# symek/facedeform

Hardware: AMD Instinct MI355X
Metric: deformed Mverts/sec at 256 ctrl pts, 1/2/4/8 MI355X vs host-CPU ref (higher is better)
Workload: dtype f32

## Files before the change

### facedeform_amd/csrc/fd_capi.hip

```cpp
#include <atomic>
#include <cstdarg>
#include <cstdio>
#include <cstdlib>
#include <cstring>
#include <new>

#include "fd_internal.h"

using namespace fd;

struct GraphKey {
    int M, kind, term, nparams;
    double params[4];
    const void *A, *rest, *rec32;
};

struct fd_batch;
struct fd_ctx {
    int device = 0;
    hipStream_t own_stream = nullptr;
    hipStream_t stream_ = nullptr;
    int eval_precision = FD_EVAL_FP32;
    int eval_variant = 0;
    int output = FD_OUTPUT_POSITION;
// ... 1631 lines not shown
    hipError_t e = launch_deform_batch(args, b->n, stream);
    if (e != hipSuccess) { batch_err(b, "launch_deform_batch failed: %s", hipGetErrorString(e)); return FD_E_DEVICE; }
    return FD_OK;
}

static int shared_applies(fd_batch *b, const char *who, float *const *d_P_out, int *ek_out)
{
    fd_ctx *c0 = b->ctxs[0];
    const int ek = eval_kind(c0);
    *ek_out = ek;
    bool fast = (ek == FD_KERNEL_THIN_PLATE || ek == FD_KERNEL_GAUSSIAN || ek == FD_KERNEL_GAUSSIAN_QNN) && round_up(c0->M, kRecPad) >= 32;
    for (int i = 0; i < b->n; ++i) {
        fd_ctx *c = b->ctxs[i];
        if (!d_P_out[i]) { batch_err(b, "%s: NULL output array for context %d", who, i); return FD_E_INVALID; }
        if (!c->built && !c->build_pending) { batch_err(b, "%s: context %d has no built model", who, i); return FD_E_NOT_BUILT; }
        if (!c->rest_src || c->rest_src != c0->rest_src || !same_model(c, c0)) {
            batch_err(b, "%s: the contexts must share one rest rig (fd_batch_set_points_dev with the "
                         "same rest array for all), kernel and term; context %d does not", who, i);
            return FD_E_INVALID;
        }
        if (c->output != c0->output) { batch_err(b, "%s: context %d has another fd_set_output setting than context 0", who, i); return FD_E_INVALID; }
        if (c->eval_precision != FD_EVAL_FP32 || c->eval_variant > 0 || record_layers(c) != 0) fast = false;
    }
    return fast ? 1 : 0;
}

static bool make_event(hipEvent_t *ev)
{
    if (*ev) return true;
    if (hipEventCreateWithFlags(ev, hipEventDisableTiming) != hipSuccess) { (void)hipGetLastError(); *ev = nullptr; return false; }
    return true;
}

static int shared_pack(fd_batch *b, hipStream_t stream, int ek, float *const *d_P_out, float *const *d_falloff_out)
{
    fd_ctx *c0 = b->ctxs[0];
    const int si = b->packed_valid ? (b->cur_set ^ 1) : 0;
    fd_batch::SharedSet &st = b->sets[si];
    SharedDeformArgs a{};
    a.N = 1; a.Mpad = round_up(c0->M, kRecPad); a.nF = b->n; a.kind = ek; a.ctiles = c0->d_tiles16;
    a.falloff_out = d_falloff_out;
    int rc;
    if (!b->lean && (rc = batch_poll(b))) return rc;
    for (int i = 0; i < b->n; ++i) {
        fd_ctx *c = b->ctxs[i];
        a.rec32[i] = c->d_rec32; a.model[i] = c->d_model; a.P_out[i] = d_P_out[i]; a.centres[i] = c->d_centres;
        if ((rc = order_after_batch(c, stream))) { batch_err(b, "context %d: %s", i, c->err); return rc; }
    }
    {
        bool one_build = c0->rig_build_id != 0;
        for (int i = 1; i < b->n && one_build; ++i) one_build = b->ctxs[i]->rig_build_id == c0->rig_build_id;
        if (one_build) for (int i = 1; i < b->n; ++i) a.centres[i] = a.centres[0];
    }
    const size_t wb = shared_wtile_bytes(a.Mpad, a.nF), fb = shared_frame_bytes(a.nF);
    if (wb > st.cap_wtiles || fb > st.cap_frames) {
        if (st.d_wtiles) (void)hipFree(st.d_wtiles);
        if (st.d_frames) (void)hipFree(st.d_frames);
        st.d_wtiles = st.d_frames = nullptr; st.cap_wtiles = st.cap_frames = 0; st.eval_pending = false;
        if (hipMalloc(&st.d_wtiles, wb) != hipSuccess || hipMalloc(&st.d_frames, fb) != hipSuccess) {
            (void)hipGetLastError();
            batch_err(b, "shared-rig evaluation: scratch allocation (%zu bytes) failed", wb + fb);
            return FD_E_NOMEM;
        }
        st.cap_wtiles = wb; st.cap_frames = fb;
    }
    if (st.eval_pending && st.eval_done && hipStreamWaitEvent(stream, st.eval_done, 0) != hipSuccess) {
        batch_err(b, "shared-rig evaluation: hipStreamWaitEvent failed: %s", hipGetErrorString(hipGetLastError()));
        return FD_E_DEVICE;
    }
    st.eval_pending = false;
    a.wtiles = st.d_wtiles; a.frames = st.d_frames;
    a.packed_ev = b->lean ? nullptr : (make_event(&st.packed_ev) ? st.packed_ev : nullptr);
    b->consumed_override = nullptr;
    a.mode = 1;
    a.M = c0->M;
    if (b->h_mismatch && hipHostGetDevicePointer((void **)&a.mismatch, b->h_mismatch, 0) != hipSuccess) { (void)hipGetLastError(); a.mismatch = nullptr; }
    hipError_t e = launch_deform_shared(a, stream);
    if (e != hipSuccess) { batch_err(b, "launch_deform_shared (pack) failed: %s", hipGetErrorString(e)); return FD_E_DEVICE; }
    b->cur_set = si;
    b->packed_valid = b->lean || st.packed_ev != nullptr;
    b->prepared = true;
    for (int i = 0; i < b->n; ++i) {
        b->prep_P_out[i] = d_P_out[i]; b->prep_fall[i] = d_falloff_out ? d_falloff_out[i] : nullptr;
        b->prep_gen[i] = b->ctxs[i]->model_gen;
    }
    b->prep_has_fall = d_falloff_out != nullptr;
    return FD_OK;
}

int fd_batch_prepare_shared(fd_batch *b, void *hip_stream, float *const *d_P_out, float *const *d_falloff_out)
{
    if (!b || !d_P_out) return FD_E_INVALID;
    fd_ctx *c0 = b->ctxs[0];
    int rc = use_device(c0);
    if (rc) { batch_err(b, "%s", c0->err); return rc; }
    hipStream_t stream = hip_stream ? (hipStream_t)hip_stream : cur_stream(c0);
    int ek = 0;
    const int applies = shared_applies(b, "fd_batch_prepare_shared", d_P_out, &ek);
    if (applies < 0) return applies;
    if (applies == 0) return FD_OK;
    return shared_pack(b, stream, ek, d_P_out, d_falloff_out);
}

int fd_batch_deform_shared_dev(fd_batch *b, void *hip_stream, int64_t N, const float *d_P_in, float *const *d_P_out,
                               const float *d_dist2, float *const *d_falloff_out, const float *d_tu,
                               const float *d_tv, const float *d_nrm, float radius2, float falloffrate)
{
    if (!b || !d_P_out) return FD_E_INVALID;
    if (N < 0 || (N > 0 && !d_P_in)) { batch_err(b, "fd_batch_deform_shared_dev: bad N / P_in"); return FD_E_INVALID; }
// ... 12 lines not shown
        rc = fd_batch_deform_dev(b, hip_stream, N, pin, d_P_out, d_dist2 ? pd2 : nullptr, d_falloff_out, d_tu ? ptu : nullptr,
                                 d_tu ? ptv : nullptr, d_tu ? pnr : nullptr, radius2, falloffrate);
        if (rc == FD_OK && make_event(&b->fallback_ev)) {
            if (hipEventRecord(b->fallback_ev, stream) != hipSuccess) { (void)hipGetLastError(); rc = FD_E_DEVICE; }
            b->packed_valid = false;
            b->consumed_override = nullptr;
        }
        return rc;
    }
    bool reuse = b->prepared && b->prep_has_fall == (d_falloff_out != nullptr);
    for (int i = 0; reuse && i < b->n; ++i)
        reuse = b->prep_P_out[i] == d_P_out[i] && (!d_falloff_out || b->prep_fall[i] == d_falloff_out[i]) &&
                b->prep_gen[i] == b->ctxs[i]->model_gen;
    if (reuse) {
        if (!b->lean && (rc = batch_poll(b))) return rc;
        if (!b->prepared) reuse = false;
        for (int i = 0; reuse && i < b->n; ++i)
            if ((rc = order_after_batch(b->ctxs[i], stream))) { batch_err(b, "context %d: %s", i, b->ctxs[i]->err); return rc; }
    }
    if (reuse) {
        fd_batch::SharedSet &ps = b->sets[b->cur_set];
        if (!b->lean && ps.packed_ev && hipStreamWaitEvent(stream, ps.packed_ev, 0) != hipSuccess) {
            batch_err(b, "fd_batch_deform_shared_dev: hipStreamWaitEvent failed: %s", hipGetErrorString(hipGetLastError()));
            return FD_E_DEVICE;
        }
    } else if ((rc = shared_pack(b, stream, ek, d_P_out, d_falloff_out))) {
        return rc;
    }
    fd_batch::SharedSet &st = b->sets[b->cur_set];
    SharedDeformArgs a{};
    a.N = N; a.P_in = d_P_in; a.dist2 = d_dist2; a.tu = d_tu; a.tv = d_tv; a.nrm = d_nrm;
    a.radius2 = radius2; a.falloffrate = falloffrate;
    a.Mpad = round_up(c0->M, kRecPad); a.nF = b->n;
    a.ctiles = c0->d_tiles16;
    a.kind = ek;
    a.falloff_out = d_falloff_out;
    for (int i = 0; i < b->n; ++i) { a.rec32[i] = b->ctxs[i]->d_rec32; a.model[i] = b->ctxs[i]->d_model; a.P_out[i] = d_P_out[i]; }
    a.wtiles = st.d_wtiles; a.frames = st.d_frames;
    a.packed_ev = nullptr;
    a.mode = 2;
    a.delta_out = c0->output == FD_OUTPUT_DISPLACEMENT;
    a.max_wgs = b->eval_cus;
    hipError_t e = launch_deform_shared(a, stream);
    if (e != hipSuccess) { batch_err(b, "launch_deform_shared failed: %s", hipGetErrorString(e)); return FD_E_DEVICE; }
    if (b->lean) {
        st.eval_done = b->ev1;
        st.eval_pending = true;
    } else if (make_event(&st.eval_ev)) {
        st.eval_done = st.eval_ev;
        if (hipEventRecord(st.eval_ev, stream) != hipSuccess) { (void)hipGetLastError(); st.eval_pending = false; }
        else st.eval_pending = true;
    } else {
        (void)hipStreamSynchronize(stream);
    }
    return FD_OK;
}

int fd_batch_deform_vectors_shared_dev(fd_batch *b, void *hip_stream, int64_t N, const float *d_P_in, float *const *d_P_out,
                                       const float *d_dist2, float *const *d_falloff_out, const float *d_tu, const float *d_tv,
                                       const float *d_nrm, float radius2, float falloffrate, const fd_batch_vectors *vec)
{
    if (!b || !d_P_out) return FD_E_INVALID;
    const char *who = "fd_batch_deform_vectors_shared_dev";
    if (vec && vec->struct_size < (int)sizeof(fd_batch_vectors)) {
        batch_err(b, "%s: vec->struct_size is %d, must be sizeof(fd_batch_vectors) = %d", who, vec->struct_size, (int)sizeof(fd_batch_vectors));
        return FD_E_INVALID;
    }
    const bool want = vec && (vec->N || vec->N_out || vec->tu || vec->tu_out || vec->tv || vec->tv_out || vec->jacobian);
    if (!want)
        return fd_batch_deform_shared_dev(b, hip_stream, N, d_P_in, d_P_out, d_dist2, d_falloff_out, d_tu, d_tv, d_nrm, radius2, falloffrate);
// ... 176 lines not shown
```

### facedeform_amd/csrc/fd_eval_shared.hip

```cpp
#include <cstdio>
#include <cstdlib>

#include <type_traits>

#include "fd_eval_common.h"

namespace fd {

namespace {

typedef _Float16 f16x8 __attribute__((ext_vector_type(8)));
typedef _Float16 f16x2 __attribute__((ext_vector_type(2)));

constexpr int kSharedThreads = 512;
constexpr int kWideWaves = 8;
constexpr size_t kSharedLdsBudget = 158 * 1024;

constexpr int kGaussShift = 10;
constexpr bool shared_dense(int nF) { return nF > 12; }
constexpr int shared_tiles(int nF) { return shared_dense(nF) ? 3 * ((nF + 15) / 16) : (nF + 3) / 4; }
constexpr int shared_slots(int nT, bool dense) { return dense ? nT / 3 * 16 : nT * 4; }

struct SharedFrame {
    float inv_scale;
    int built;
    int pad[2];
    float *P_out, *falloff_out;
};
static_assert(sizeof(SharedFrame) == 32, "frame record");

struct SharedOut {
    float *P_out[kMaxBatch];
// ... 536 lines not shown
                }
                if (fout) __builtin_nontemporal_store(fall, (float FD_GLOBAL *)((char FD_GLOBAL *)(fout + 4ull * (uint64_t)vbase) + off4));
                store_pos3_nt(dstP, base[0] + disp[0] * fall, base[1] + disp[1] * fall, base[2] + disp[2] * fall);
            }
        }
        FD_SSTAMP(3)
    };
    int grp = blockIdx.x;
    bool built_here = true;
#pragma unroll
    for (int q = 0; q < kTabRegs; ++q) {
        const int idx = 64 * q + lane;
        if (idx < kSlots * 8 && (idx & 7) == 1) built_here = built_here && tab[q] != 0u;
    }
    if (p.fast && __all(built_here)) {
        const int nfull = (int)(p.N / kSharedThreads);
        for (; grp < nfull; grp += gridDim.x) do_group(grp, std::true_type{});
    }
    for (; grp < ngroups; grp += gridDim.x) do_group(grp, std::false_type{});
    if (stamp && lane == 0) {
        for (int q = 0; q < 4; ++q) p.stamps[wave * 8 + q] = st_acc[q];
    }
#undef FD_SSTAMP
}


typedef float f32x16 __attribute__((ext_vector_type(16)));
constexpr bool shared_wide(int nF, int kind) { (void)kind; return nF > 16; }
constexpr int kWideSlots = 32;
constexpr int wide_slots(int nF) { return (nF + 3) / 4 * 4; }
constexpr int wide_tiles(int nslot) { return (3 * nslot + 31) / 32; }
constexpr int wide_w16(int nt) { return nt * 2 * 2 * 64; }

__global__ __launch_bounds__(256) void k_pack_shared_wide(const SharedSlots slots, const SharedOut out, int nF, int nslot, int Mpad,
                                                           uint4 *wtiles, SharedFrame *frames, const MfmaTileH *ctiles, int gauss, int layout)
{
    const int kb = blockIdx.x, T = blockIdx.y, nkb = gridDim.x, NT = gridDim.y;
    const int w16 = wide_w16(NT);
    const size_t poly_at = (size_t)nkb * w16, copy_at = poly_at + (size_t)NT * 64;
    if (T == 0) {
        uint2 *dst = reinterpret_cast<uint2 *>(wtiles + copy_at) + (size_t)kb * 128;
        if (gauss) {
            if (threadIdx.x < 32) {
                const int centre = 32 * kb + (int)threadIdx.x;
                wtiles[copy_at + (size_t)kb * 64 + threadIdx.x] =
                    centre < Mpad ? *reinterpret_cast<const uint4 *>(&slots.rec32[0][centre]) : make_uint4(0u, 0u, 0u, 0u);
            }
        } else if (layout == 1) {
            if (threadIdx.x < 64) {
                const int lane = threadIdx.x, h = lane >> 5, r = lane & 31;
                const int tile = 2 * kb + (r >> 4);
                uint4 v = make_uint4(0u, 0u, 0u, 0u);
                if (tile < Mpad / 16) {
                    const unsigned *a0 = ctiles[tile].a[16 * (2 * h) + (r & 15)], *a1 = ctiles[tile].a[16 * (2 * h + 1) + (r & 15)];
                    v = make_uint4(a0[0], a0[1], a1[0], a1[1]);
                }
                wtiles[copy_at + (size_t)kb * 64 + lane] = v;
            }
        } else if (threadIdx.x < 128) {
            const int i = threadIdx.x >> 6, lane = threadIdx.x & 63, h = lane >> 5, r = lane & 31;
            const int tile = 2 * kb + (r >> 4);
            uint2 v = make_uint2(0u, 0u);
            if (tile < Mpad / 16) { const unsigned *a = ctiles[tile].a[16 * (2 * i + h) + (r & 15)]; v = make_uint2(a[0], a[1]); }
            dst[threadIdx.x] = v;
        }
        if (kb == 0 && threadIdx.x == 255) {
            const float *nn = slots.model[0]->norm32;
            wtiles[copy_at + (size_t)nkb * 64] = make_uint4(__float_as_uint(nn[0]), __float_as_uint(nn[1]), __float_as_uint(nn[2]), __float_as_uint(nn[3]));
        }
    }
    __shared__ float s_scale[kWideSlots];
    {
        const int f = threadIdx.x >> 3, l = threadIdx.x & 7;
        float m = 0.f;
        if (f < nslot) {
            m = slots.model[f]->wmax32;
        }
        for (int off = 4; off >= 1; off >>= 1) m = fmaxf(m, __shfl_xor(m, off));
        const bool same_rig = (kb == 0 && T == 0) ? rig_matches(slots, f, nslot, l, 8) : true;
        if (l == 0) {
            int k = 0;
            if (m > 0.f && m < INFINITY) k = 13 - (__builtin_amdgcn_frexp_expf(m) - 1);
            k = k < -100 ? -100 : (k > 100 ? 100 : k);
            s_scale[f] = ldexpf(1.f, k);
            if (kb == 0 && T == 0) {
                SharedFrame fr;
                fr.inv_scale = ldexpf(1.f, -k - (gauss ? kGaussShift : 0));
                fr.built = (f < nslot && same_rig && slots.model[f]->terminationtype == 1) ? 1 : 0;
                fr.pad[0] = fr.pad[1] = 0;
                fr.P_out = f < nslot ? out.P_out[f] : nullptr;
                fr.falloff_out = f < nslot ? out.falloff_out[f] : nullptr;
                frames[f] = fr;
            }
        }
    }
    __syncthreads();
    if (threadIdx.x >= 128) return;
    const int s = threadIdx.x >> 6, lane = threadIdx.x & 63, h = lane >> 5;
    int f, c;
    if (layout == 1) {
        const int rho = lane & 31, k = 16 * T + 4 * (rho >> 3) + (rho & 3);
        f = 2 * (k / 3) + ((rho >> 2) & 1); c = k % 3;
    } else {
        const int row = 32 * T + (lane & 31);
        f = row / 3; c = row % 3;
    }
    const bool live = f < nslot;
    const float sc = live ? s_scale[f] : 0.f;
    f16x8 hi, lo;
#pragma unroll
    for (int m = 0; m < 8; ++m) {
        const int centre = 32 * kb + 8 * (2 * s + (m >> 2)) + 4 * h + (m & 3);
        float w = 0.f;
        if (live && centre < Mpad) {
            const Rec32 r = slots.rec32[f][centre];
            w = (c == 0 ? r.wx : (c == 1 ? r.wy : r.wz)) * sc;
        }
        const _Float16 hh = (_Float16)w;
        hi[m] = hh;
        lo[m] = (_Float16)(w - (float)hh);
    }
    uint4 *dst = wtiles + (size_t)kb * w16 + (size_t)((T * 2 + s) * 2) * 64;
    dst[lane] = __builtin_bit_cast(uint4, hi);
    dst[64 + lane] = __builtin_bit_cast(uint4, lo);
    if (kb == 0 && s == 0) {
        f16x8 pt;
#pragma unroll
        for (int m = 0; m < 8; ++m) {
            const int coef = h == 0 ? (m < 5 ? m : m - 4) : (m == 0 ? 4 : (m < 6 ? m - 1 : -1));
            const bool want_lo = h == 1 && m >= 1;
            float w = 0.f;
            if (live && coef >= 0) w = slots.model[f]->poly32[5 * c + coef] * sc;
            const _Float16 hh = (_Float16)w;
            pt[m] = want_lo ? (_Float16)(w - (float)hh) : hh;
        }
        wtiles[poly_at + (size_t)T * 64 + lane] = __builtin_bit_cast(uint4, pt);
    }
}

constexpr int kWideVpm = 3;
constexpr int kW1Vpm = 3;

template <bool GAUSS, int NT, int NSLOT>
__global__ __launch_bounds__(64 * kWideWaves) __attribute__((amdgpu_waves_per_eu(kWideWaves / 4, kWideWaves / 4)))
void k_deform32_tps_shared_wide(const SharedParams p, int ngroups)
{
    constexpr int WAVES = kWideWaves, THREADS = 64 * WAVES;
    static_assert(NSLOT % 4 == 0 && NSLOT <= kWideSlots && 3 * NSLOT <= 32 * NT, "frame slots in fours, three rows each");
    constexpr int kWideW16 = wide_w16(NT);
    constexpr int TV = 2;
    constexpr int kSlots = kWideSlots;
    extern __shared__ __attribute__((aligned(16))) char smem[];
    SharedFrame *s_frames = reinterpret_cast<SharedFrame *>(smem);
    uint4 *s_poly = reinterpret_cast<uint4 *>(smem + sizeof(SharedFrame) * (size_t)kSlots);
    uint2 *s_ct = reinterpret_cast<uint2 *>(s_poly + NT * 64);
    uint4 *s_w = reinterpret_cast<uint4 *>(s_ct + (size_t)128 * p.kchunk);
    uint64_t *s_ftab = reinterpret_cast<uint64_t *>(s_w + (size_t)kWideW16 * p.kchunk);
    unsigned *s_ticket = reinterpret_cast<unsigned *>(s_ftab + 512);
    const int tid = threadIdx.x;
    const int lane = tid & 63;
    const int wave = __builtin_amdgcn_readfirstlane(tid >> 6);
    const int h = lane >> 5, j = lane & 31;
    const float n0 = p.norm[0], n1 = p.norm[1], n2 = p.norm[2];
    const float inv_s = p.norm[3];
    const bool resident = p.nkb <= p.kchunk;
    const unsigned long long st_t0 = p.stamps ? __builtin_amdgcn_s_memtime() : 0, st_r0 = p.stamps ? __builtin_amdgcn_s_memrealtime() : 0;
    f32x16 zero16;
#pragma unroll
    for (int r = 0; r < 16; ++r) zero16[r] = 0.f;

// ... 347 lines not shown
    int ru = dynamic ? round_taken : 0;
    nxt = load_raw(unit_group(u) < ngroups ? unit_global(u) : 0, std::false_type{});
    settle(nxt);
    if (fast_ok) {
        while (unit_group(u) < nfull) {
            const int un = next_unit(u);
            const int run = dynamic ? round_taken : ru + 1;
            do_group(u, un, ru, std::true_type{});
            u = un; ru = run;
        }
    }
    while (unit_group(u) < ngroups) {
        const int un = next_unit(u);
        const int run = dynamic ? round_taken : ru + 1;
        do_group(u, un, ru, std::false_type{});
        u = un; ru = run;
    }
    if (stamp && lane == 0 && wave < 8) {
        for (int q = 0; q < 4; ++q) p.stamps[wave * 8 + q] = st_acc[q];
        p.stamps[wave * 8 + 4] = __builtin_amdgcn_s_memtime() - st_t0;
        p.stamps[wave * 8 + 5] = __builtin_amdgcn_s_memrealtime() - st_r0;
    }
    if (p.stamps != nullptr && lane == 0 && wave < 8 && blockIdx.x < kMaxCUs) {
        p.stamps[64 + ((size_t)blockIdx.x * 8 + wave) * 2] = st_r0;
        p.stamps[64 + ((size_t)blockIdx.x * 8 + wave) * 2 + 1] = __builtin_amdgcn_s_memrealtime();
    }
#undef FD_SSTAMP
}

constexpr int kW1Waves = 12;
constexpr int kW1Unit = 32;
constexpr size_t w1_fixed_lds(int nt) { return sizeof(SharedFrame) * (size_t)kWideSlots + 32 * 16 + (size_t)nt * 64 * 16 + 256 * sizeof(uint64_t) + 16; }

template <bool GAUSS, int NT, int NSLOT>
__global__ __launch_bounds__(64 * kW1Waves) __attribute__((amdgpu_waves_per_eu(kW1Waves / 4, kW1Waves / 4)))
void k_deform32_shared_w1(const SharedParams p, int ngroups)
{
    constexpr int WAVES = kW1Waves, THREADS = 64 * WAVES;
    constexpr int NLF = NSLOT / 2;
    constexpr int NFQ = (NSLOT + 7) / 8;
    static_assert(NSLOT % 4 == 0 && NSLOT <= kWideSlots && 3 * NLF <= 16 * NT, "frame slots in fours, three rows each, half of them per lane half");
    constexpr int kW16 = wide_w16(NT);
    extern __shared__ __attribute__((aligned(16))) char smem[];
    SharedFrame *s_frames = reinterpret_cast<SharedFrame *>(smem);
    uint4 *s_ptab = reinterpret_cast<uint4 *>(smem + sizeof(SharedFrame) * (size_t)kWideSlots);
    uint4 *s_poly = s_ptab + 32;
    uint64_t *s_ftab = reinterpret_cast<uint64_t *>(s_poly + NT * 64);
    unsigned *s_ticket = reinterpret_cast<unsigned *>(s_ftab + 256);
    uint4 *s_ct = reinterpret_cast<uint4 *>(s_ticket + 4);
    uint4 *s_w = s_ct + (size_t)64 * p.kchunk;
    const int tid = threadIdx.x;
    const int lane = tid & 63;
    const int wave = __builtin_amdgcn_readfirstlane(tid >> 6);
    const int h = lane >> 5, j = lane & 31;
    const float n0 = p.norm[0], n1 = p.norm[1], n2 = p.norm[2];
    const float inv_s = p.norm[3];
    f32x16 zero16;
#pragma unroll
    for (int r = 0; r < 16; ++r) zero16[r] = 0.f;

    auto stage_model = [&]() {
        const int nk = p.nkb;
        for (int q = tid; q < nk * 64; q += THREADS) s_ct[q] = reinterpret_cast<const uint4 *>(p.ctiles)[q];
        const u32x4 *src = reinterpret_cast<const u32x4 *>(p.wtiles);
        u32x4 *dst = reinterpret_cast<u32x4 *>(s_w);
        const int n16 = nk * kW16;
        int q = tid;
        for (; q + 7 * THREADS < n16; q += 8 * THREADS) {
            const u32x4 v0 = src[q], v1 = src[q + THREADS], v2 = src[q + 2 * THREADS], v3 = src[q + 3 * THREADS];
            const u32x4 v4 = src[q + 4 * THREADS], v5 = src[q + 5 * THREADS], v6 = src[q + 6 * THREADS], v7 = src[q + 7 * THREADS];
            dst[q] = v0; dst[q + THREADS] = v1; dst[q + 2 * THREADS] = v2; dst[q + 3 * THREADS] = v3;
            dst[q + 4 * THREADS] = v4; dst[q + 5 * THREADS] = v5; dst[q + 6 * THREADS] = v6; dst[q + 7 * THREADS] = v7;
        }
        for (; q < n16; q += THREADS) dst[q] = src[q];
        __syncthreads();
    };

    {
        const uint4 *src = reinterpret_cast<const uint4 *>(p.frames);
        uint4 *dst = reinterpret_cast<uint4 *>(s_frames);
        for (int q = tid; q < kWideSlots * (int)(sizeof(SharedFrame) / 16); q += THREADS) dst[q] = src[q];
        const uint4 *psrc = p.wtiles + (size_t)p.nkb * kW16;
        for (int q = tid; q < NT * 64; q += THREADS) s_poly[q] = psrc[q];
        if (tid == 0) *s_ticket = 0u;
        if (tid < 32) {
            const SharedFrame fr = p.frames[tid < NSLOT ? tid : NSLOT - 1];
            const uint64_t po = (uint64_t)fr.P_out;
            s_ptab[tid] = make_uint4((unsigned)po, (unsigned)(po >> 32), __float_as_uint(fr.inv_scale), (unsigned)fr.built);
        }
        if (p.fast && tid < NFQ * 64) {
            const int f = 8 * (tid >> 6) + ((tid & 63) >> 3);
            s_ftab[tid] = (uint64_t)p.frames[f < NSLOT ? f : NSLOT - 1].falloff_out + 16u * (unsigned)(tid & 7);
        }
    }
    stage_model();

    struct UnitRaw { float p[3]; float d2; };
    const int whole_rounds = ngroups / (int)gridDim.x;
    const int pool0 = whole_rounds * (int)gridDim.x * WAVES, total_units = ngroups * WAVES;
    auto unit_global = [&](int u) -> int {
        if (u < WAVES * whole_rounds) return ((int)blockIdx.x + (u / WAVES) * (int)gridDim.x) * WAVES + (u % WAVES);
        const int q = u - WAVES * whole_rounds;
        return q < 2 * WAVES ? pool0 + (int)blockIdx.x + q * (int)gridDim.x : total_units;
    };
    auto unit_group = [&](int u) -> int { const int g = unit_global(u); return g < total_units ? (g / WAVES) : ngroups; };
    auto next_unit = [&](int u) {
        (void)u;
        unsigned v = 0;
        if (lane == 0) v = __hip_atomic_fetch_add(s_ticket, 1u, __ATOMIC_RELAXED, __HIP_MEMORY_SCOPE_WORKGROUP);
        return (int)__builtin_amdgcn_readfirstlane(v);
    };
    auto load_raw = [&](int gu, auto fastTag) {
        constexpr bool FAST = decltype(fastTag)::value;
        UnitRaw r;
        const int64_t vi = (int64_t)gu * kW1Unit + j;
        const int64_t vc = vi < p.N ? vi : p.N - 1;
        if constexpr (FAST) {
            const char *pb = reinterpret_cast<const char *>(p.P_in) + (size_t)(12u * (unsigned)vc);
            r.p[0] = __builtin_nontemporal_load(reinterpret_cast<const float *>(pb)); r.p[1] = __builtin_nontemporal_load(reinterpret_cast<const float *>(pb + 4));
            r.p[2] = __builtin_nontemporal_load(reinterpret_cast<const float *>(pb + 8));
            r.d2 = 0.f;
        } else {
            r.p[0] = __builtin_nontemporal_load(&p.P_in[3 * vc]); r.p[1] = __builtin_nontemporal_load(&p.P_in[3 * vc + 1]);
            r.p[2] = __builtin_nontemporal_load(&p.P_in[3 * vc + 2]);
            r.d2 = p.dist2 ? p.dist2[vc] : 0.f;
        }
        return r;
    };
// ... 204 lines not shown
                    for (int c = 0; c < 3; ++c) gm[r][c] = u3[r] * u3[c] + v3[r] * v3[c] + n3[r] * n3[c];
#pragma unroll
                for (int c = 0; c < 3; ++c) {
                    a1[c] = u3[0] * gm[0][c] + u3[1] * gm[1][c] + u3[2] * gm[2][c];
                    a2[c] = v3[0] * gm[0][c] + v3[1] * gm[1][c] + v3[2] * gm[2][c];
                }
                normalize3(a1[0], a1[1], a1[2]);
                normalize3(a2[0], a2[1], a2[2]);
            }
        }
#pragma unroll
        for (int lf = 0; lf < NLF; ++lf) {
            const int f = 2 * lf + h;
            if (f >= p.nF || !doit) continue;
            const SharedFrame fr = s_frames[f];
            Pos3 FD_GLOBAL *dstP = (Pos3 FD_GLOBAL *)as_global(fr.P_out) + i;
            if (!fr.built) {
                if (p.delta) store_pos3(dstP, 0.f, 0.f, 0.f);
                else if (fr.P_out != p.P_in) store_pos3(dstP, pos[0], pos[1], pos[2]);
                continue;
            }
            float disp[3] = {accf(3 * lf) * fr.inv_scale, accf(3 * lf + 1) * fr.inv_scale, accf(3 * lf + 2) * fr.inv_scale};
            if (p.tu) {
                const float da1 = disp[0] * a1[0] + disp[1] * a1[1] + disp[2] * a1[2];
                const float da2 = disp[0] * a2[0] + disp[1] * a2[1] + disp[2] * a2[2];
#pragma unroll
                for (int c = 0; c < 3; ++c) disp[c] = a1[c] * da1 + a2[c] * da2;
            }
            if (fr.falloff_out) __builtin_nontemporal_store(fall, (float FD_GLOBAL *)as_global(fr.falloff_out) + i);
            store_pos3_nt(dstP, base[0] + disp[0] * fall, base[1] + disp[1] * fall, base[2] + disp[2] * fall);
        }
    };
    bool built_here = true;
    if (lane < NSLOT) built_here = p.frames[lane].built != 0;
    const bool fast_ok = p.fast && __all(built_here);
    const int nfull = (int)(p.N / (kW1Unit * WAVES));
    int u = next_unit(0);
    nxt = load_raw(unit_group(u) < ngroups ? unit_global(u) : 0, std::false_type{});
    settle(nxt);
    if (fast_ok) {
        while (unit_group(u) < nfull) {
            const int un = next_unit(u);
            do_unit(u, un, std::true_type{});
            u = un;
        }
    }
    while (unit_group(u) < ngroups) {
        const int un = next_unit(u);
        do_unit(u, un, std::false_type{});
        u = un;
    }
#ifdef FD_TUNING
    if (stamp && lane == 0 && wave < 16) {
        for (int q = 0; q < 3; ++q) p.stamps[wave * 8 + q] = st_acc[q];
        p.stamps[wave * 8 + 3] = (unsigned long long)uc;
        p.stamps[wave * 8 + 4] = __builtin_amdgcn_s_memtime() - st_t0;
        p.stamps[wave * 8 + 5] = __builtin_amdgcn_s_memrealtime() - st_r0;
    }
#endif
#undef FD_W1STAMP
}
}

hipError_t launch_deform_shared(const SharedDeformArgs &a, hipStream_t stream)
{
    if (a.N <= 0 || a.nF <= 0) return hipSuccess;
    if (a.nF > kMaxBatch || a.Mpad % 16 != 0) return hipErrorInvalidValue;
    const int ntiles = a.Mpad / 16, nkb = (ntiles + 1) / 2;
    const bool gauss = a.kind != FD_KERNEL_THIN_PLATE;
    const bool wide = shared_wide(a.nF, a.kind);
    const bool dense = shared_dense(a.nF);
    const int nT = shared_tiles(a.nF);
    const int wslot = wide_slots(a.nF), wNT = wide_tiles(wslot);
    const int nslot = wide ? wslot : shared_slots(nT, dense);
    SharedSlots slots{};
    SharedOut out{};
    for (int f = 0; f < kMaxBatch; ++f) {
        const int q = f < a.nF ? f : a.nF - 1;
        slots.rec32[f] = a.rec32[q]; slots.model[f] = a.model[q]; slots.centres[f] = a.centres[q];
        out.P_out[f] = a.P_out[q]; out.falloff_out[f] = a.falloff_out ? a.falloff_out[q] : nullptr;
    }
    slots.M = a.M; slots.nreal = a.nF; slots.mismatch = a.mismatch;
    const bool w1 = wide && (kSharedLdsBudget - w1_fixed_lds(wNT)) / ((size_t)1024 + (size_t)wide_w16(wNT) * 16) >= (size_t)nkb;
    if (a.mode != 2) {
        if (wide)
            hipLaunchKernelGGL(k_pack_shared_wide, dim3(nkb, wNT), dim3(256), 0, stream, slots, out, a.nF, wslot, a.Mpad, (uint4 *)a.wtiles,
                               (SharedFrame *)a.frames, a.ctiles, gauss ? 1 : 0, w1 ? 1 : 0);
        else
            hipLaunchKernelGGL(k_pack_shared, dim3(nkb, nT), dim3(256), 0, stream, slots, out, nslot, a.Mpad, dense ? 1 : 0, (uint4 *)a.wtiles,
                               (SharedFrame *)a.frames, a.ctiles, gauss ? 1 : 0);
        if (a.packed_ev) {
            hipError_t e = hipEventRecord(a.packed_ev, stream);
            if (e != hipSuccess) return e;
        }
        if (a.mode == 1) return hipGetLastError();
    }
    SharedParams p{};
    p.N = a.N; p.P_in = a.P_in; p.dist2 = a.dist2; p.tu = a.tu; p.tv = a.tv; p.nrm = a.nrm;
    p.radius2 = a.radius2; p.falloffrate = a.falloffrate; p.delta = a.delta_out;
    p.ntiles = ntiles; p.nkb = nkb; p.nF = a.nF; p.nT = nT;
    if (wide) {
        const uint4 *copy = (const uint4 *)a.wtiles + (size_t)nkb * wide_w16(wNT) + (size_t)wNT * 64;
        p.ctiles = reinterpret_cast<const MfmaTileH *>(copy);
        p.norm = reinterpret_cast<const float *>(copy + (size_t)nkb * 64);
    } else {
        const uint4 *copy = (const uint4 *)a.wtiles + (size_t)nkb * nT * 128 + (size_t)nT * 64;
        p.ctiles = reinterpret_cast<const MfmaTileH *>(copy);
        p.norm = reinterpret_cast<const float *>(copy + (size_t)2 * nkb * (sizeof(MfmaTileH) / 16));
    }
    p.wtiles = (const uint4 *)a.wtiles; p.frames = (const SharedFrame *)a.frames;
    {
        bool fast = !a.delta_out && a.dist2 == nullptr && a.tu == nullptr && a.radius2 > 0.f && a.falloff_out != nullptr &&
                    a.N < ((int64_t)1 << 28) && 4 * (nslot - a.nF) <= a.nF;
        for (int f = 0; fast && f < a.nF; ++f) fast = a.falloff_out[f] != nullptr && a.P_out[f] != nullptr && ((uintptr_t)a.falloff_out[f] & 15) == 0;
        p.fast = fast ? 1 : 0;
    }
#ifdef FD_TUNING
    static unsigned long long *d_stamps = nullptr;
    static const bool want_stamps = tuning_env("FD_SHARED_STAMPS") != nullptr;
    constexpr size_t kStampWords = 64 + (size_t)kMaxCUs * 8 * 2;
    if (want_stamps && !d_stamps) (void)hipMalloc((void **)&d_stamps, kStampWords * sizeof(unsigned long long));
    if (want_stamps && d_stamps) (void)hipMemsetAsync(d_stamps, 0, kStampWords * sizeof(unsigned long long), stream);
    p.stamps = want_stamps ? d_stamps : nullptr;
#else
    p.stamps = nullptr;
#endif
    const size_t fixed = w1 ? w1_fixed_lds(wNT) :
                         wide ? sizeof(SharedFrame) * (size_t)kWideSlots + (size_t)wNT * 64 * 16 + 512 * sizeof(uint64_t) + 16
                              : sizeof(SharedFrame) * (size_t)shared_slots(nT, dense) + (size_t)nT * 64 * 16;
    const size_t per_kb = wide ? (size_t)1024 + (size_t)wide_w16(wNT) * 16 : 2 * sizeof(MfmaTileH) + (size_t)nT * 128 * 16;
    int kchunk = (int)((kSharedLdsBudget - fixed) / per_kb);
    if (kchunk < 1) return hipErrorInvalidValue;
    if (kchunk > nkb) kchunk = nkb;
    p.kchunk = kchunk;
    const size_t lds = fixed + per_kb * (size_t)kchunk;
    const int64_t per = w1 ? kW1Unit * kW1Waves : wide ? 64 * kWideWaves : kSharedThreads / 64 * 64;
    const int64_t ngroups = (a.N + per - 1) / per;
    const int64_t max_wgs = a.max_wgs > 0 ? (a.max_wgs < 4096 ? a.max_wgs : 4096) : (int64_t)device_cus();
    const unsigned grid = (unsigned)(ngroups < max_wgs ? ngroups : max_wgs);
#define FD_SHARED_CASE(NTV, DNS, GSS)                                                                                \
    {                                                                                                                \
        static LdsAttrOnce once;                                                                                     \
        hipError_t e = once.ensure((const void *)k_deform32_tps_shared<NTV, DNS, GSS>, 160 * 1024);                  \
        if (e != hipSuccess) return e;                                                                               \
        hipLaunchKernelGGL((k_deform32_tps_shared<NTV, DNS, GSS>), dim3(grid), dim3(kSharedThreads), lds, stream, p, (int)ngroups); \
    }
#define FD_SHARED_KIND(NTV, DNS) { if (gauss) FD_SHARED_CASE(NTV, DNS, true) else FD_SHARED_CASE(NTV, DNS, false) }
#define FD_WIDE_CASE(GSS, NTW, NSL)                                                                                  \
    {                                                                                                                \
        static LdsAttrOnce once;                                                                                     \
        hipError_t e = once.ensure((const void *)k_deform32_tps_shared_wide<GSS, NTW, NSL>, 160 * 1024); \
        if (e != hipSuccess) return e;                                                                               \
        hipLaunchKernelGGL((k_deform32_tps_shared_wide<GSS, NTW, NSL>), dim3(grid), dim3(64 * kWideWaves), lds, stream, p, (int)ngroups); \
    }
#define FD_WIDE_KIND(NTW, NSL) { if (gauss) FD_WIDE_CASE(true, NTW, NSL) else FD_WIDE_CASE(false, NTW, NSL) }
#define FD_W1_CASE(GSS, NTW, NSL)                                                                                    \
    {                                                                                                                \
        static LdsAttrOnce once;                                                                                     \
        hipError_t e = once.ensure((const void *)k_deform32_shared_w1<GSS, NTW, NSL>, 160 * 1024);                   \
        if (e != hipSuccess) return e;                                                                               \
        hipLaunchKernelGGL((k_deform32_shared_w1<GSS, NTW, NSL>), dim3(grid), dim3(64 * kW1Waves), lds, stream, p, (int)ngroups); \
    }
#define FD_W1_KIND(NTW, NSL) { if (gauss) FD_W1_CASE(true, NTW, NSL) else FD_W1_CASE(false, NTW, NSL) }
    if (w1) {
        if (wslot == 20) FD_W1_KIND(2, 20)
        else if (wslot == 24) FD_W1_KIND(3, 24)
        else if (wslot == 28) FD_W1_KIND(3, 28)
        else if (wslot == 32) FD_W1_KIND(3, 32)
        else return hipErrorInvalidValue;
    } else if (wide) {
        if (wslot == 20) FD_WIDE_KIND(2, 20)
        else if (wslot == 24) FD_WIDE_KIND(3, 24)
        else if (wslot == 28) FD_WIDE_KIND(3, 28)
        else if (wslot == 32) FD_WIDE_KIND(3, 32)
        else return hipErrorInvalidValue;
    } else if (dense) {
        if (nT == 3) FD_SHARED_KIND(3, true)
        else return hipErrorInvalidValue;
    } else {
        if (nT == 1) FD_SHARED_KIND(1, false)
        else if (nT == 2) FD_SHARED_KIND(2, false)
        else if (nT == 3) FD_SHARED_KIND(3, false)
        else return hipErrorInvalidValue;
    }
#undef FD_SHARED_KIND
#undef FD_SHARED_CASE
#undef FD_WIDE_CASE
#undef FD_WIDE_KIND
#undef FD_W1_CASE
#undef FD_W1_KIND
#ifdef FD_TUNING
    if (want_stamps && d_stamps) {
        static unsigned long long h[kStampWords];
        (void)hipStreamSynchronize(stream);
        if (hipMemcpy(h, d_stamps, sizeof(h), hipMemcpyDeviceToHost) == hipSuccess) {
            if (w1) {
                fprintf(stderr, "[w1 stamps, shader cycles per wave of workgroup 0: load+poly | K loop | epilogue | units | whole (counts, 100 MHz ticks)]\n");
                for (int w = 0; w < kW1Waves; ++w)
                    fprintf(stderr, "   wave %2d: %8llu %8llu %8llu  units %llu  whole %llu counts in %llu ticks = %.3f GHz\n", w, h[w * 8], h[w * 8 + 1], h[w * 8 + 2], h[w * 8 + 3],
                            h[w * 8 + 4], h[w * 8 + 5], h[w * 8 + 5] ? (double)h[w * 8 + 4] / (double)h[w * 8 + 5] * 0.1 : 0.0);
            } else if (wide) {
                unsigned long long t0 = ~0ull, t1 = 0;
                const unsigned sgrid = grid < kMaxCUs ? grid : kMaxCUs;
                for (unsigned b = 0; b < sgrid * 8; ++b) if (h[64 + 2 * b]) { t0 = h[64 + 2 * b] < t0 ? h[64 + 2 * b] : t0; t1 = h[65 + 2 * b] > t1 ? h[65 + 2 * b] : t1; }
                fprintf(stderr, "[shared stamps: %u workgroups, first entry to last exit %.1f us; per workgroup (entry, exit) in us after the first entry:]\n", grid, (t1 - t0) * 0.01);
                for (unsigned b = 0; b < sgrid; ++b) {
                    unsigned long long a = ~0ull, z = 0;
                    for (int w = 0; w < 8; ++w) if (h[64 + 2 * (b * 8 + w)]) { a = h[64 + 2 * (b * 8 + w)] < a ? h[64 + 2 * (b * 8 + w)] : a; z = h[65 + 2 * (b * 8 + w)] > z ? h[65 + 2 * (b * 8 + w)] : z; }
                    fprintf(stderr, "%s%5.1f-%5.1f", b % 8 ? "  " : "\n   ", (a - t0) * 0.01, (z - t0) * 0.01);
                }
                fprintf(stderr, "\n");
            }
            if (!w1) fprintf(stderr, "[shared stamps, shader cycles per wave of workgroup 0: load+poly | K loop | transposes | per-vertex + frames]\n");
            for (int w = 0; w < 8 && !w1; ++w)
                fprintf(stderr, "   wave %d: %8llu %8llu %8llu %8llu   (whole: %llu counts in %llu reference ticks)\n", w, h[w * 8], h[w * 8 + 1], h[w * 8 + 2], h[w * 8 + 3],
                        h[w * 8 + 4], h[w * 8 + 5]);
        }
    }
#endif
    return hipGetLastError();
}

// ... 41 lines not shown
```

### facedeform_amd/csrc/fd_internal.h

```cpp
#pragma once

#include <hip/hip_runtime.h>
#include <stdint.h>

#include "../../include/facedeform_hip.h"

#include "fd_tuning.h"

namespace fd {

#define FD_GLOBAL __attribute__((address_space(1)))
typedef double FD_GLOBAL gdouble;
typedef const double FD_GLOBAL gcdouble;
template <typename T> __host__ __device__ __forceinline__ T FD_GLOBAL *as_global(T *p) { return (T FD_GLOBAL *)p; }

struct Rec32 {
    float cx, cy, cz, s;
    float wx, wy, wz, pad;
};
struct Rec64 {
    double cx, cy, cz, s;
    double wx, wy, wz, pad;
};

// ... 141 lines not shown
    const MfmaTile *tiles;
    const MfmaTileH *tiles16;
    const DevModel *model;
    int precision, variant;
    int layers;
    int delta_out;
};
hipError_t launch_deform(const DeformArgs &a, hipStream_t stream);
struct VectorArgs {
    const float *N, *tu, *tv;
    float *N_out, *tu_out, *tv_out;
    float *jacobian;
};
hipError_t launch_vectors(const DeformArgs &a, const VectorArgs &v, hipStream_t stream);
hipError_t launch_deform_batch(const DeformArgs *a, int n, hipStream_t stream);
struct SharedDeformArgs {
    int64_t N;
    const float *P_in;
    const float *dist2;
    const float *tu, *tv, *nrm;
    float radius2, falloffrate;
    int Mpad, nF;
    int kind;
    const MfmaTileH *ctiles;
    const Rec32 *rec32[kMaxBatch];
    const DevModel *model[kMaxBatch];
    float *P_out[kMaxBatch];
    float *const *falloff_out;
    void *wtiles, *frames;
    hipEvent_t packed_ev;
    int mode;
    int delta_out;
    int max_wgs;
    const double *centres[kMaxBatch];
    int M;
    int *mismatch;
};
hipError_t launch_deform_shared(const SharedDeformArgs &a, hipStream_t stream);
size_t shared_wtile_bytes(int Mpad, int nF);
size_t shared_frame_bytes(int nF);
const char *shared_kernel_name(int Mpad, int nF, int kind);
struct SharedPacking {
    int layout, ntiles;
    size_t poly_at, copy_at, norm_at;
};
SharedPacking shared_packing(int Mpad, int nF);
struct SharedVectorArgs {
    int64_t N;
    const float *P_in, *dist2, *tu, *tv, *nrm;
    float radius2, falloffrate;
    int Mpad, nF, kind;
    const float *vN, *vtu, *vtv;
    float *N_out[kMaxBatch], *tu_out[kMaxBatch], *tv_out[kMaxBatch], *jacobian[kMaxBatch];
    const void *wtiles, *frames;
    int max_wgs;
};
hipError_t launch_vectors_shared(const SharedVectorArgs &a, hipStream_t stream);
const char *shared_vectors_kernel_name(int Mpad, int nF, int kind);
hipError_t launch_capture_islands(const float *d_P, int64_t N, const int64_t *d_offsets, const int *d_neighbours,
                                  const float *d_rig, int M, int max_edges, unsigned char *d_mask, hipStream_t stream);
hipError_t launch_capture_dist2(const float *d_P, int64_t N, const unsigned char *d_mask, const float *d_tri, int T,
                                float radius2, int dofalloff, float *d_dist2, hipStream_t stream);
const char *deform_kernel_name(int kind, int precision, int variant);

}
```

Baseline: 64610.

## Fuse shared-rig weight packing into the w1 deform kernel for lean batches

For lean batches using the w1 wide kernel with a shared rig, the separate pack kernel launch is skipped. Each workgroup of the deform kernel builds the scaled fp16 hi/lo weight tiles, poly words, centre operands and frame records straight into LDS from the model records. This removes a kernel launch and a global scratch round-trip per pack. In exchange, every workgroup repeats the packing work and the rig-match check is assumed true.

```diff
diff --git a/facedeform_amd/csrc/fd_capi.hip b/facedeform_amd/csrc/fd_capi.hip
--- a/facedeform_amd/csrc/fd_capi.hip
+++ b/facedeform_amd/csrc/fd_capi.hip
@@ -1687,26 +1687,39 @@
     return true;
 }
 
+static void shared_sources(fd_batch *b, SharedDeformArgs &a)
+{
+    fd_ctx *c0 = b->ctxs[0];
+    for (int i = 0; i < b->n; ++i) {
+        fd_ctx *c = b->ctxs[i];
+        a.rec32[i] = c->d_rec32; a.model[i] = c->d_model; a.centres[i] = c->d_centres;
+    }
+    bool one_build = c0->rig_build_id != 0;
+    for (int i = 1; i < b->n && one_build; ++i) one_build = b->ctxs[i]->rig_build_id == c0->rig_build_id;
+    if (one_build) for (int i = 1; i < b->n; ++i) a.centres[i] = a.centres[0];
+    a.M = c0->M;
+    a.ctiles = c0->d_tiles16;
+    a.mismatch = nullptr;
+    if (b->h_mismatch && hipHostGetDevicePointer((void **)&a.mismatch, b->h_mismatch, 0) != hipSuccess) { (void)hipGetLastError(); a.mismatch = nullptr; }
+    a.direct = b->lean ? 1 : 0;
+}
+
 static int shared_pack(fd_batch *b, hipStream_t stream, int ek, float *const *d_P_out, float *const *d_falloff_out)
 {
     fd_ctx *c0 = b->ctxs[0];
     const int si = b->packed_valid ? (b->cur_set ^ 1) : 0;
     fd_batch::SharedSet &st = b->sets[si];
     SharedDeformArgs a{};
-    a.N = 1; a.Mpad = round_up(c0->M, kRecPad); a.nF = b->n; a.kind = ek; a.ctiles = c0->d_tiles16;
+    a.N = 1; a.Mpad = round_up(c0->M, kRecPad); a.nF = b->n; a.kind = ek;
     a.falloff_out = d_falloff_out;
     int rc;
     if (!b->lean && (rc = batch_poll(b))) return rc;
     for (int i = 0; i < b->n; ++i) {
         fd_ctx *c = b->ctxs[i];
-        a.rec32[i] = c->d_rec32; a.model[i] = c->d_model; a.P_out[i] = d_P_out[i]; a.centres[i] = c->d_centres;
+        a.P_out[i] = d_P_out[i];
         if ((rc = order_after_batch(c, stream))) { batch_err(b, "context %d: %s", i, c->err); return rc; }
     }
-    {
-        bool one_build = c0->rig_build_id != 0;
-        for (int i = 1; i < b->n && one_build; ++i) one_build = b->ctxs[i]->rig_build_id == c0->rig_build_id;
-        if (one_build) for (int i = 1; i < b->n; ++i) a.centres[i] = a.centres[0];
-    }
+    shared_sources(b, a);
     const size_t wb = shared_wtile_bytes(a.Mpad, a.nF), fb = shared_frame_bytes(a.nF);
     if (wb > st.cap_wtiles || fb > st.cap_frames) {
         if (st.d_wtiles) (void)hipFree(st.d_wtiles);
@@ -1728,8 +1741,6 @@
     a.packed_ev = b->lean ? nullptr : (make_event(&st.packed_ev) ? st.packed_ev : nullptr);
     b->consumed_override = nullptr;
     a.mode = 1;
-    a.M = c0->M;
-    if (b->h_mismatch && hipHostGetDevicePointer((void **)&a.mismatch, b->h_mismatch, 0) != hipSuccess) { (void)hipGetLastError(); a.mismatch = nullptr; }
     hipError_t e = launch_deform_shared(a, stream);
     if (e != hipSuccess) { batch_err(b, "launch_deform_shared (pack) failed: %s", hipGetErrorString(e)); return FD_E_DEVICE; }
     b->cur_set = si;
@@ -1808,10 +1819,11 @@
     a.N = N; a.P_in = d_P_in; a.dist2 = d_dist2; a.tu = d_tu; a.tv = d_tv; a.nrm = d_nrm;
     a.radius2 = radius2; a.falloffrate = falloffrate;
     a.Mpad = round_up(c0->M, kRecPad); a.nF = b->n;
-    a.ctiles = c0->d_tiles16;
     a.kind = ek;
     a.falloff_out = d_falloff_out;
+    a.ctiles = c0->d_tiles16;
     for (int i = 0; i < b->n; ++i) { a.rec32[i] = b->ctxs[i]->d_rec32; a.model[i] = b->ctxs[i]->d_model; a.P_out[i] = d_P_out[i]; }
+    if (b->lean) shared_sources(b, a);
     a.wtiles = st.d_wtiles; a.frames = st.d_frames;
     a.packed_ev = nullptr;
     a.mode = 2;
diff --git a/facedeform_amd/csrc/fd_eval_shared.hip b/facedeform_amd/csrc/fd_eval_shared.hip
--- a/facedeform_amd/csrc/fd_eval_shared.hip
+++ b/facedeform_amd/csrc/fd_eval_shared.hip
@@ -1,3 +1,4 @@
+#include <cstddef>
 #include <cstdio>
 #include <cstdlib>
 
@@ -600,6 +601,80 @@
 constexpr int wide_tiles(int nslot) { return (3 * nslot + 31) / 32; }
 constexpr int wide_w16(int nt) { return nt * 2 * 2 * 64; }
 
+__device__ __forceinline__ uint4 wide_d2_operand(const MfmaTileH *ctiles, int Mpad, int kb, int lane)
+{
+    const int h = lane >> 5, r = lane & 31;
+    const int tile = 2 * kb + (r >> 4);
+    uint4 v = make_uint4(0u, 0u, 0u, 0u);
+    if (tile < Mpad / 16) {
+        const unsigned *a0 = ctiles[tile].a[16 * (2 * h) + (r & 15)], *a1 = ctiles[tile].a[16 * (2 * h + 1) + (r & 15)];
+        v = make_uint4(a0[0], a0[1], a1[0], a1[1]);
+    }
+    return v;
+}
+__device__ __forceinline__ uint4 wide_gauss_centre(const Rec32 *rec0, int Mpad, int kb, int t)
+{
+    const int centre = 32 * kb + t;
+    return centre < Mpad ? *reinterpret_cast<const uint4 *>(&rec0[centre]) : make_uint4(0u, 0u, 0u, 0u);
+}
+__device__ __forceinline__ int wide_scale_exp(float m)
+{
+    int k = 0;
+    if (m > 0.f && m < INFINITY) k = 13 - (__builtin_amdgcn_frexp_expf(m) - 1);
+    return k < -100 ? -100 : (k > 100 ? 100 : k);
+}
+__device__ __forceinline__ SharedFrame wide_frame_record(const SharedSlots &slots, const SharedOut &out, int f, int nslot, int gauss,
+                                                         bool same_rig, int k)
+{
+    SharedFrame fr;
+    fr.inv_scale = ldexpf(1.f, -k - (gauss ? kGaussShift : 0));
+    fr.built = (f < nslot && same_rig && slots.model[f]->terminationtype == 1) ? 1 : 0;
+    fr.pad[0] = fr.pad[1] = 0;
+    fr.P_out = f < nslot ? out.P_out[f] : nullptr;
+    fr.falloff_out = f < nslot ? out.falloff_out[f] : nullptr;
+    return fr;
+}
+__device__ __forceinline__ void wide_row(int layout, int T, int lane, int &f, int &c)
+{
+    if (layout == 1) {
+        const int rho = lane & 31, k = 16 * T + 4 * (rho >> 3) + (rho & 3);
+        f = 2 * (k / 3) + ((rho >> 2) & 1); c = k % 3;
+    } else {
+        const int row = 32 * T + (lane & 31);
+        f = row / 3; c = row % 3;
+    }
+}
+__device__ __forceinline__ void wide_weight_pair(const SharedSlots &slots, int f, int c, bool live, float sc, int Mpad, int kb, int s, int h,
+                                                 uint4 &hi16, uint4 &lo16)
+{
+    f16x8 hi, lo;
+#pragma unroll
+    for (int m = 0; m < 8; ++m) {
+        const int centre = 32 * kb + 8 * (2 * s + (m >> 2)) + 4 * h + (m & 3);
+        float w = 0.f;
+        if (live && centre < Mpad) w = (&slots.rec32[f][centre].wx)[c] * sc;
+        const _Float16 hh = (_Float16)w;
+        hi[m] = hh;
+        lo[m] = (_Float16)(w - (float)hh);
+    }
+    hi16 = __builtin_bit_cast(uint4, hi);
+    lo16 = __builtin_bit_cast(uint4, lo);
+}
+__device__ __forceinline__ uint4 wide_poly_word(const SharedSlots &slots, int f, int c, bool live, float sc, int h)
+{
+    f16x8 pt;
+#pragma unroll
+    for (int m = 0; m < 8; ++m) {
+        const int coef = h == 0 ? (m < 5 ? m : m - 4) : (m == 0 ? 4 : (m < 6 ? m - 1 : -1));
+        const bool want_lo = h == 1 && m >= 1;
+        float w = 0.f;
+        if (live && coef >= 0) w = slots.model[f]->poly32[5 * c + coef] * sc;
+        const _Float16 hh = (_Float16)w;
+        pt[m] = want_lo ? (_Float16)(w - (float)hh) : hh;
+    }
+    return __builtin_bit_cast(uint4, pt);
+}
+
 __global__ __launch_bounds__(256) void k_pack_shared_wide(const SharedSlots slots, const SharedOut out, int nF, int nslot, int Mpad,
                                                            uint4 *wtiles, SharedFrame *frames, const MfmaTileH *ctiles, int gauss, int layout)
 {
@@ -609,22 +684,9 @@
     if (T == 0) {
         uint2 *dst = reinterpret_cast<uint2 *>(wtiles + copy_at) + (size_t)kb * 128;
         if (gauss) {
-            if (threadIdx.x < 32) {
-                const int centre = 32 * kb + (int)threadIdx.x;
-                wtiles[copy_at + (size_t)kb * 64 + threadIdx.x] =
-                    centre < Mpad ? *reinterpret_cast<const uint4 *>(&slots.rec32[0][centre]) : make_uint4(0u, 0u, 0u, 0u);
-            }
+            if (threadIdx.x < 32) wtiles[copy_at + (size_t)kb * 64 + threadIdx.x] = wide_gauss_centre(slots.rec32[0], Mpad, kb, threadIdx.x);
         } else if (layout == 1) {
-            if (threadIdx.x < 64) {
-                const int lane = threadIdx.x, h = lane >> 5, r = lane & 31;
-                const int tile = 2 * kb + (r >> 4);
-                uint4 v = make_uint4(0u, 0u, 0u, 0u);
-                if (tile < Mpad / 16) {
-                    const unsigned *a0 = ctiles[tile].a[16 * (2 * h) + (r & 15)], *a1 = ctiles[tile].a[16 * (2 * h + 1) + (r & 15)];
-                    v = make_uint4(a0[0], a0[1], a1[0], a1[1]);
-                }
-                wtiles[copy_at + (size_t)kb * 64 + lane] = v;
-            }
+            if (threadIdx.x < 64) wtiles[copy_at + (size_t)kb * 64 + threadIdx.x] = wide_d2_operand(ctiles, Mpad, kb, threadIdx.x);
         } else if (threadIdx.x < 128) {
             const int i = threadIdx.x >> 6, lane = threadIdx.x & 63, h = lane >> 5, r = lane & 31;
             const int tile = 2 * kb + (r >> 4);
@@ -647,63 +709,24 @@
         for (int off = 4; off >= 1; off >>= 1) m = fmaxf(m, __shfl_xor(m, off));
         const bool same_rig = (kb == 0 && T == 0) ? rig_matches(slots, f, nslot, l, 8) : true;
         if (l == 0) {
-            int k = 0;
-            if (m > 0.f && m < INFINITY) k = 13 - (__builtin_amdgcn_frexp_expf(m) - 1);
-            k = k < -100 ? -100 : (k > 100 ? 100 : k);
+            const int k = wide_scale_exp(m);
             s_scale[f] = ldexpf(1.f, k);
-            if (kb == 0 && T == 0) {
-                SharedFrame fr;
-                fr.inv_scale = ldexpf(1.f, -k - (gauss ? kGaussShift : 0));
-                fr.built = (f < nslot && same_rig && slots.model[f]->terminationtype == 1) ? 1 : 0;
-                fr.pad[0] = fr.pad[1] = 0;
-                fr.P_out = f < nslot ? out.P_out[f] : nullptr;
-                fr.falloff_out = f < nslot ? out.falloff_out[f] : nullptr;
-                frames[f] = fr;
-            }
+            if (kb == 0 && T == 0) frames[f] = wide_frame_record(slots, out, f, nslot, gauss, same_rig, k);
         }
     }
     __syncthreads();
     if (threadIdx.x >= 128) return;
     const int s = threadIdx.x >> 6, lane = threadIdx.x & 63, h = lane >> 5;
     int f, c;
-    if (layout == 1) {
-        const int rho = lane & 31, k = 16 * T + 4 * (rho >> 3) + (rho & 3);
-        f = 2 * (k / 3) + ((rho >> 2) & 1); c = k % 3;
-    } else {
-        const int row = 32 * T + (lane & 31);
-        f = row / 3; c = row % 3;
-    }
+    wide_row(layout, T, lane, f, c);
     const bool live = f < nslot;
     const float sc = live ? s_scale[f] : 0.f;
-    f16x8 hi, lo;
-#pragma unroll
-    for (int m = 0; m < 8; ++m) {
-        const int centre = 32 * kb + 8 * (2 * s + (m >> 2)) + 4 * h + (m & 3);
-        float w = 0.f;
-        if (live && centre < Mpad) {
-            const Rec32 r = slots.rec32[f][centre];
-            w = (c == 0 ? r.wx : (c == 1 ? r.wy : r.wz)) * sc;
-        }
-        const _Float16 hh = (_Float16)w;
-        hi[m] = hh;
-        lo[m] = (_Float16)(w - (float)hh);
-    }
+    uint4 hi, lo;
+    wide_weight_pair(slots, f, c, live, sc, Mpad, kb, s, h, hi, lo);
     uint4 *dst = wtiles + (size_t)kb * w16 + (size_t)((T * 2 + s) * 2) * 64;
-    dst[lane] = __builtin_bit_cast(uint4, hi);
-    dst[64 + lane] = __builtin_bit_cast(uint4, lo);
-    if (kb == 0 && s == 0) {
-        f16x8 pt;
-#pragma unroll
-        for (int m = 0; m < 8; ++m) {
-            const int coef = h == 0 ? (m < 5 ? m : m - 4) : (m == 0 ? 4 : (m < 6 ? m - 1 : -1));
-            const bool want_lo = h == 1 && m >= 1;
-            float w = 0.f;
-            if (live && coef >= 0) w = slots.model[f]->poly32[5 * c + coef] * sc;
-            const _Float16 hh = (_Float16)w;
-            pt[m] = want_lo ? (_Float16)(w - (float)hh) : hh;
-        }
-        wtiles[poly_at + (size_t)T * 64 + lane] = __builtin_bit_cast(uint4, pt);
-    }
+    dst[lane] = hi;
+    dst[64 + lane] = lo;
+    if (kb == 0 && s == 0) wtiles[poly_at + (size_t)T * 64 + lane] = wide_poly_word(slots, f, c, live, sc, h);
 }
 
 constexpr int kWideVpm = 3;
@@ -1117,9 +1140,16 @@
 constexpr int kW1Unit = 32;
 constexpr size_t w1_fixed_lds(int nt) { return sizeof(SharedFrame) * (size_t)kWideSlots + 32 * 16 + (size_t)nt * 64 * 16 + 256 * sizeof(uint64_t) + 16; }
 
-template <bool GAUSS, int NT, int NSLOT>
+struct SharedDirect {
+    SharedSlots slots;
+    SharedOut out;
+    const MfmaTileH *ctiles;
+    int Mpad;
+};
+struct SharedStaged { int unused; };
+template <bool GAUSS, int NT, int NSLOT, bool DIRECT>
 __global__ __launch_bounds__(64 * kW1Waves) __attribute__((amdgpu_waves_per_eu(kW1Waves / 4, kW1Waves / 4)))
-void k_deform32_shared_w1(const SharedParams p, int ngroups)
+void k_deform32_shared_w1(const SharedParams p, int ngroups, const std::conditional_t<DIRECT, SharedDirect, SharedStaged> d)
 {
     constexpr int WAVES = kW1Waves, THREADS = 64 * WAVES;
     constexpr int NLF = NSLOT / 2;
@@ -1161,7 +1191,50 @@
         __syncthreads();
     };
 
-    {
+    if constexpr (DIRECT) {
+        auto frame_scale = [&](int f) { return __int_as_float(s_frames[f].pad[0]); };
+        if (tid < kWideSlots) {
+            const int f = tid;
+            const int k = wide_scale_exp(f < NSLOT ? d.slots.model[f]->wmax32 : 0.f);
+            SharedFrame fr = wide_frame_record(d.slots, d.out, f, NSLOT, GAUSS ? 1 : 0, true, k);
+            fr.pad[0] = __float_as_int(ldexpf(1.f, k));
+            s_frames[f] = fr;
+        }
+        if (tid == THREADS - 1) *s_ticket = 0u;
+        for (int q = tid; q < p.nkb * 64; q += THREADS) {
+            if constexpr (GAUSS) { if ((q & 63) < 32) s_ct[q] = wide_gauss_centre(d.slots.rec32[0], d.Mpad, q >> 6, q & 63); }
+            else s_ct[q] = wide_d2_operand(d.ctiles, d.Mpad, q >> 6, q & 63);
+        }
+        __syncthreads();
+        if (tid < 32) {
+            const SharedFrame fr = s_frames[tid < NSLOT ? tid : NSLOT - 1];
+            const uint64_t po = (uint64_t)fr.P_out;
+            s_ptab[tid] = make_uint4((unsigned)po, (unsigned)(po >> 32), __float_as_uint(fr.inv_scale), (unsigned)fr.built);
+        }
+        if (p.fast && tid < NFQ * 64) {
+            const int f = 8 * (tid >> 6) + ((tid & 63) >> 3);
+            s_ftab[tid] = (uint64_t)s_frames[f < NSLOT ? f : NSLOT - 1].falloff_out + 16u * (unsigned)(tid & 7);
+        }
+        for (int q = tid; q < p.nkb * NT * 128; q += THREADS) {
+            const int ln = q & 63, s = (q >> 6) & 1, T = (q >> 7) % NT, kb = (q >> 7) / NT;
+            int f, c;
+            wide_row(1, T, ln, f, c);
+            const bool live = f < NSLOT;
+            uint4 hi, lo;
+            wide_weight_pair(d.slots, f, c, live, live ? frame_scale(f) : 0.f, d.Mpad, kb, s, ln >> 5, hi, lo);
+            uint4 *dst = s_w + (size_t)kb * kW16 + (size_t)((T * 2 + s) * 2) * 64;
+            dst[ln] = hi;
+            dst[64 + ln] = lo;
+        }
+        if (tid >= THREADS - NT * 64) {
+            const int q = tid - (THREADS - NT * 64), T = q >> 6, ln = q & 63;
+            int f, c;
+            wide_row(1, T, ln, f, c);
+            const bool live = f < NSLOT;
+            s_poly[q] = wide_poly_word(d.slots, f, c, live, live ? frame_scale(f) : 0.f, ln >> 5);
+        }
+        __syncthreads();
+    } else {
         const uint4 *src = reinterpret_cast<const uint4 *>(p.frames);
         uint4 *dst = reinterpret_cast<uint4 *>(s_frames);
         for (int q = tid; q < kWideSlots * (int)(sizeof(SharedFrame) / 16); q += THREADS) dst[q] = src[q];
@@ -1177,8 +1250,9 @@
             const int f = 8 * (tid >> 6) + ((tid & 63) >> 3);
             s_ftab[tid] = (uint64_t)p.frames[f < NSLOT ? f : NSLOT - 1].falloff_out + 16u * (unsigned)(tid & 7);
         }
-    }
-    stage_model();
+        stage_model();
+    }
+    (void)stage_model;
 
     struct UnitRaw { float p[3]; float d2; };
     const int whole_rounds = ngroups / (int)gridDim.x;
@@ -1449,7 +1523,7 @@
         }
     };
     bool built_here = true;
-    if (lane < NSLOT) built_here = p.frames[lane].built != 0;
+    if (lane < NSLOT) built_here = (DIRECT ? s_frames[lane].built : p.frames[lane].built) != 0;
     const bool fast_ok = p.fast && __all(built_here);
     const int nfull = (int)(p.N / (kW1Unit * WAVES));
     int u = next_unit(0);
@@ -1499,6 +1573,9 @@
     }
     slots.M = a.M; slots.nreal = a.nF; slots.mismatch = a.mismatch;
     const bool w1 = wide && (kSharedLdsBudget - w1_fixed_lds(wNT)) / ((size_t)1024 + (size_t)wide_w16(wNT) * 16) >= (size_t)nkb;
+    bool direct = a.direct && w1;
+    for (int f = 1; direct && f < a.nF; ++f) direct = a.centres[f] == a.centres[0];
+    if (direct && a.mode == 1) return hipSuccess;
     if (a.mode != 2) {
         if (wide)
             hipLaunchKernelGGL(k_pack_shared_wide, dim3(nkb, wNT), dim3(256), 0, stream, slots, out, a.nF, wslot, a.Mpad, (uint4 *)a.wtiles,
@@ -1526,6 +1603,12 @@
         p.norm = reinterpret_cast<const float *>(copy + (size_t)2 * nkb * (sizeof(MfmaTileH) / 16));
     }
     p.wtiles = (const uint4 *)a.wtiles; p.frames = (const SharedFrame *)a.frames;
+    SharedDirect dir{};
+    if (direct) {
+        dir.slots = slots; dir.out = out; dir.ctiles = a.ctiles; dir.Mpad = a.Mpad;
+        p.ctiles = nullptr; p.wtiles = nullptr; p.frames = nullptr;
+        p.norm = reinterpret_cast<const float *>(reinterpret_cast<const char *>(a.model[0]) + offsetof(DevModel, norm32));
+    }
     {
         bool fast = !a.delta_out && a.dist2 == nullptr && a.tu == nullptr && a.radius2 > 0.f && a.falloff_out != nullptr &&
                     a.N < ((int64_t)1 << 28) && 4 * (nslot - a.nF) <= a.nF;
@@ -1571,14 +1654,15 @@
         hipLaunchKernelGGL((k_deform32_tps_shared_wide<GSS, NTW, NSL>), dim3(grid), dim3(64 * kWideWaves), lds, stream, p, (int)ngroups); \
     }
 #define FD_WIDE_KIND(NTW, NSL) { if (gauss) FD_WIDE_CASE(true, NTW, NSL) else FD_WIDE_CASE(false, NTW, NSL) }
-#define FD_W1_CASE(GSS, NTW, NSL)                                                                                    \
+#define FD_W1_CASE(GSS, NTW, NSL, DIR, ARG)                                                                          \
     {                                                                                                                \
         static LdsAttrOnce once;                                                                                     \
-        hipError_t e = once.ensure((const void *)k_deform32_shared_w1<GSS, NTW, NSL>, 160 * 1024);                   \
+        hipError_t e = once.ensure((const void *)k_deform32_shared_w1<GSS, NTW, NSL, DIR>, 160 * 1024);              \
         if (e != hipSuccess) return e;                                                                               \
-        hipLaunchKernelGGL((k_deform32_shared_w1<GSS, NTW, NSL>), dim3(grid), dim3(64 * kW1Waves), lds, stream, p, (int)ngroups); \
-    }
-#define FD_W1_KIND(NTW, NSL) { if (gauss) FD_W1_CASE(true, NTW, NSL) else FD_W1_CASE(false, NTW, NSL) }
+        hipLaunchKernelGGL((k_deform32_shared_w1<GSS, NTW, NSL, DIR>), dim3(grid), dim3(64 * kW1Waves), lds, stream, p, (int)ngroups, ARG); \
+    }
+#define FD_W1_FORM(GSS, NTW, NSL) { if (direct) FD_W1_CASE(GSS, NTW, NSL, true, dir) else FD_W1_CASE(GSS, NTW, NSL, false, SharedStaged{0}) }
+#define FD_W1_KIND(NTW, NSL) { if (gauss) FD_W1_FORM(true, NTW, NSL) else FD_W1_FORM(false, NTW, NSL) }
     if (w1) {
         if (wslot == 20) FD_W1_KIND(2, 20)
         else if (wslot == 24) FD_W1_KIND(3, 24)
@@ -1605,6 +1689,7 @@
 #undef FD_WIDE_CASE
 #undef FD_WIDE_KIND
 #undef FD_W1_CASE
+#undef FD_W1_FORM
 #undef FD_W1_KIND
 #ifdef FD_TUNING
     if (want_stamps && d_stamps) {
diff --git a/facedeform_amd/csrc/fd_internal.h b/facedeform_amd/csrc/fd_internal.h
--- a/facedeform_amd/csrc/fd_internal.h
+++ b/facedeform_amd/csrc/fd_internal.h
@@ -197,6 +197,7 @@
     int mode;
     int delta_out;
     int max_wgs;
+    int direct;
     const double *centres[kMaxBatch];
     int M;
     int *mismatch;
```

Result: slower. 61740 (-4.4%).
